# VaibhavKamat/Performance-Comparison-of-TensorFlow-PyTorch-and-their-Distributed-Counterparts

Hardware: AMD Instinct MI355X
Metric: resnet50_train_images_per_sec (higher is better)
Workload: dtype bf16; 1 GPU; model=resnet50, global_batch=256, per_gpu_batch=256, image_size=224, num_classes=1000, parallelism=dp1, impl=hip, optimizer=sgd_momentum, hipgraph=False, ddp_force=False, grad_allreduce_dtype=fp32, lr_warmup_steps=5

## Files before the change

performance-comparison-of-tensorflow-pytorch-and-their-distributed-counterparts_amd/csrc/bnr_stream.h:

```cpp
#pragma once
#include "igemm.h"

namespace pcmp {

inline Knob kn_bnr_stream("bnr_stream", 1);
inline Knob kn_bnr_stream_wgs("bnr_stream_wgs", 256);

template <int BN, int GK, bool FOLD, bool DUAL>
__global__ void __launch_bounds__(256, 2) bnr_stream_kernel(const IgemmParams p, int groups) {
  constexpr int BM = 32, NTHR = 256;
  constexpr int KB = GK / 64;
  constexpr int A_IMG = BM * GK * 2;
  constexpr int STAGE = A_IMG * (FOLD ? 2 : 1);
  constexpr int W_BYTES = BN * GK * 2;
  constexpr int CS = BN + 8;
  constexpr int C_BYTES = BM * CS * 4;
  constexpr int CPR = BN / 8;
  constexpr int NCH = BM * BN / 8 / NTHR;
  constexpr int RPP = NTHR / CPR;
  constexpr int NS = DUAL ? 3 : 2;
  constexpr int NWT = BN / 32;
  constexpr int NAI = A_IMG / 1024 / 4;
  constexpr int NWI = W_BYTES / 1024 / 4;
  constexpr int NEL = NCH * (DUAL ? 4 : 3);
// ... 212 lines not shown
        u &= mfx ? kz : kbits;
        const float g0 = __uint_as_float(u << 16), g1 = __uint_as_float(u & 0xffff0000u);
        sm[0][2 * q] += g0;
        sm[0][2 * q + 1] += g1;
        sm[1][2 * q] += g0 * fmaf(xa, ka[2 * q], kb[2 * q]);
        sm[1][2 * q + 1] += g1 * fmaf(xb, ka[2 * q + 1], kb[2 * q + 1]);
        if constexpr (DUAL) {
          const unsigned x2w = q == 0 ? eX2[S][k].x : q == 1 ? eX2[S][k].y : q == 2 ? eX2[S][k].z : eX2[S][k].w;
          sm[2][2 * q] += g0 * fmaf(__uint_as_float(x2w << 16), ka2[2 * q], kb2[2 * q]);
          sm[2][2 * q + 1] += g1 * fmaf(__uint_as_float(x2w & 0xffff0000u), ka2[2 * q + 1], kb2[2 * q + 1]);
        }
        ov[q] = u;
      }
      const size_t o = (size_t)(pt * BM + row) * p.gn + n0 + c8 * 8;
      *reinterpret_cast<uint4*>(out + o) = uint4{ov[0], ov[1], ov[2], ov[3]};
    }
  };
  int j = 0;
  for (; j + 1 < nmine; j += 2) {
    tile(std::integral_constant<int, 0>{}, j);
    tile(std::integral_constant<int, 1>{}, j + 1);
  }
  if (j < nmine) tile(std::integral_constant<int, 0>{}, j);

  __syncthreads();
  float* red = reinterpret_cast<float*>(sS);
#pragma unroll
  for (int q = 0; q < NS; ++q) {
    *reinterpret_cast<f32x4*>(red + (r0 * NS + q) * BN + c8 * 8) = f32x4{sm[q][0], sm[q][1], sm[q][2], sm[q][3]};
    *reinterpret_cast<f32x4*>(red + (r0 * NS + q) * BN + c8 * 8 + 4) = f32x4{sm[q][4], sm[q][5], sm[q][6], sm[q][7]};
  }
  __syncthreads();
  for (int i = tid; i < NS * BN; i += NTHR) {
    const int q = i / BN, c = i - q * BN;
    float t = 0.f;
    for (int r = 0; r < RPP; ++r) t += red[(r * NS + q) * BN + c];
    float* st = p.stats + (size_t)grp * 2 * p.gn;
    if (q == 0) {
      st[n0 + c] = t;
      if constexpr (DUAL) p.stats2[(size_t)grp * 2 * p.gn + n0 + c] = t;
    } else if (q == 1) {
      st[p.gn + n0 + c] = t;
    } else {
      p.stats2[(size_t)grp * 2 * p.gn + p.gn + n0 + c] = t;
    }
  }
}

static bool use_bnr_stream(const IgemmParams& p) {
  if (!kn_bnr_stream.get() || !p.bn_x || p.R != 1 || p.S != 1 || p.stride != 1 || p.pad != 0) return false;
  if (!(p.gk == 64 || p.gk == 128 || p.gk == 256) || p.gn % 64 || p.gm % 32) return false;
  if (!p.bn_mbits && !(p.bn_msc && !p.bn_mask)) return false;
  if (p.relu) return false;
  if ((p.fold_x ? 2 : 1) * p.gk >= p.gn) return false;
  return (int64_t)p.gm * p.gn * 2 < (1ll << 31) && (int64_t)p.gm * p.gk * 2 < (1ll << 31);
}

static int bnr_stream_bn(const IgemmParams& p) { return p.gn == 64 ? 64 : 128; }

static int bnr_stream_groups(const IgemmParams& p) {
  const int ntn = p.gn / bnr_stream_bn(p);
  const int npt = p.gm / 32;
  return std::max(1, std::min(npt, std::max(1, kn_bnr_stream_wgs.get() / ntn)));
}

template <int BN, int GK, bool FOLD, bool DUAL>
static void launch_bnr_stream_cfg(IgemmParams& p, hipStream_t st) {
  constexpr int BM = 32;
  const int ntn = p.gn / BN;
  const int groups = bnr_stream_groups(p);
  TORCH_CHECK(p.stats && p.stats_cap >= groups && (!DUAL || p.stats2), "bnr_stream: partial-stats buffers");
  constexpr size_t stage = (size_t)BM * GK * 2 * (FOLD ? 2 : 1);
  constexpr size_t red = (size_t)(256 / (BN / 8)) * (DUAL ? 3 : 2) * BN * 4;
  constexpr size_t body = 2 * stage + (size_t)BM * (BN + 8) * 4 + (FOLD ? 3 * GK * 4 : 0);
  constexpr size_t smem = (size_t)BN * GK * 2 + std::max(body, red);
  static_assert(smem <= 160 * 1024, "bnr_stream: LDS");
  launch_lds<bnr_stream_kernel<BN, GK, FOLD, DUAL>>(dim3(groups * ntn), dim3(256), smem, st, p, groups);
}

static void launch_bnr_stream(IgemmParams& p, hipStream_t st) {
  const bool fold = p.fold_x != nullptr, dual = p.bn_x2 != nullptr;
  const int BN = bnr_stream_bn(p);
#define PCMP_BNRS(B, G)                                                                      \
  do {                                                                                      \
    if (fold) {                                                                             \
      if (dual) launch_bnr_stream_cfg<B, G, true, true>(p, st);                             \
      else launch_bnr_stream_cfg<B, G, true, false>(p, st);                                 \
    } else {                                                                                \
      if (dual) launch_bnr_stream_cfg<B, G, false, true>(p, st);                            \
      else launch_bnr_stream_cfg<B, G, false, false>(p, st);                                \
    }                                                                                       \
  } while (0)
  if (BN == 64) {
    if (p.gk == 64) PCMP_BNRS(64, 64); else if (p.gk == 128) PCMP_BNRS(64, 128); else PCMP_BNRS(64, 256);
  } else {
    if (p.gk == 64) PCMP_BNRS(128, 64); else if (p.gk == 128) PCMP_BNRS(128, 128); else PCMP_BNRS(128, 256);
  }
#undef PCMP_BNRS
}

}

namespace pcmp {

inline Knob kn_fwd_stream("fwd_stream", 1);
inline Knob kn_fwd_stream_wgs("fwd_stream_wgs", 512);

// ... 214 lines not shown
```

performance-comparison-of-tensorflow-pytorch-and-their-distributed-counterparts_amd/csrc/igemm.h:

```cpp
#pragma once
#include "igemm_plan.h"

namespace pcmp {

static unsigned tensor_bytes(const at::Tensor& t) {
  const int64_t b = t.numel() * t.element_size();
  TORCH_CHECK(b < (1ll << 31), "igemm: operand larger than 2 GiB (buffer-resource range)");
  return (unsigned)b;
}

static void fill_geometry(IgemmParams& p, int N, int H, int W, int C, int K, int R, int S,
                          int stride, int pad) {
  p.N = N; p.H = H; p.W = W; p.C = C; p.K = K; p.R = R; p.S = S;
  p.stride = stride; p.pad = pad;
  p.P = (H + 2 * pad - R) / stride + 1;
  p.Q = (W + 2 * pad - S) / stride + 1;
  p.fd_PQ = make_fastdiv(p.P * p.Q);
  p.fd_Q = make_fastdiv(p.Q);
  p.fd_HW = make_fastdiv(H * W);
  p.fd_W = make_fastdiv(W);
  p.dH = H; p.dW = W; p.offy = pad; p.offx = pad; p.sub = 0; p.oph = 0; p.opw = 0;
  p.bias = nullptr; p.resid = nullptr; p.aux = nullptr; p.stats = nullptr; p.stats2 = nullptr;
  p.bn_mask = nullptr; p.bn_x = nullptr; p.bn_mean = nullptr; p.bn_istd = nullptr;
  p.bn_x2 = nullptr; p.bn_mean2 = nullptr; p.bn_istd2 = nullptr; p.bn_msc = nullptr; p.bn_msh = nullptr;
  p.bn_mbits = nullptr;
  p.stats_cap = 0;
  p.relu = 0; p.alpha = 1.f; p.accumulate = 0; p.nsplit = 1;
  p.fold_x = nullptr; p.fold_coef = nullptr; p.fold_lds = 0;
  p.act_sc = nullptr; p.act_sh = nullptr;
  p.resid_sub = 0; p.rs_H2 = 0; p.rs_W2 = 0;
}

std::vector<at::Tensor> conv_fwd(const at::Tensor& x, const at::Tensor& w, int64_t stride, int64_t pad,
                                 const c10::optional<at::Tensor>& bias,
                                 const c10::optional<at::Tensor>& resid, bool relu, bool want_stats,
                                 const c10::optional<at::Tensor>& in_scale, const c10::optional<at::Tensor>& in_shift);
std::vector<std::string> plan_candidates(const at::Tensor& x, const at::Tensor& w, int64_t stride, int64_t pad,
                                         const c10::optional<at::Tensor>& bias, const c10::optional<at::Tensor>& resid,
                                         bool relu);
std::vector<at::Tensor> linear_gelu_fwd(const at::Tensor& x, const at::Tensor& w, const c10::optional<at::Tensor>& bias);
at::Tensor conv_dgrad(const at::Tensor& dy, const at::Tensor& w, int64_t H, int64_t W, int64_t stride, int64_t pad,
                      const c10::optional<at::Tensor>& resid, const c10::optional<at::Tensor>& wt);
at::Tensor linear_dgrad_gelu(const at::Tensor& dy, const at::Tensor& w, const at::Tensor& u,
                             const c10::optional<at::Tensor>& wt);
std::vector<at::Tensor> conv_dgrad_bnr(const at::Tensor& dy, const at::Tensor& w, int64_t H, int64_t W,
                                       int64_t stride, int64_t pad, const c10::optional<at::Tensor>& resid,
                                       const c10::optional<at::Tensor>& ymask, const at::Tensor& x,
                                       const at::Tensor& mean, const at::Tensor& invstd,
                                       const c10::optional<at::Tensor>& x2, const c10::optional<at::Tensor>& mean2,
                                       const c10::optional<at::Tensor>& invstd2, const c10::optional<at::Tensor>& mscale,
                                       const c10::optional<at::Tensor>& mshift, const c10::optional<at::Tensor>& wt,
                                       const c10::optional<at::Tensor>& ymask_bits,
                                       const c10::optional<at::Tensor>& fold_x,
                                       const c10::optional<at::Tensor>& fold_coef, bool resid_sub);
void conv_wgrad(const at::Tensor& dy, const at::Tensor& x, at::Tensor out, int64_t R, int64_t S,
                int64_t stride, int64_t pad, bool accumulate, const c10::optional<at::Tensor>& fold_x,
                const c10::optional<at::Tensor>& fold_coef, const c10::optional<at::Tensor>& in_scale,
                const c10::optional<at::Tensor>& in_shift);
std::vector<at::Tensor> conv1x1_bwd_fused(const at::Tensor& g, const c10::optional<at::Tensor>& fold_x,
                                          const c10::optional<at::Tensor>& fold_coef, const at::Tensor& wt,
                                          const at::Tensor& z, const at::Tensor& scale, const at::Tensor& shift,
                                          const at::Tensor& mean, const at::Tensor& invstd, at::Tensor dw,
                                          bool accumulate);

}
```

performance-comparison-of-tensorflow-pytorch-and-their-distributed-counterparts_amd/csrc/igemm_dgrad.hip:

```cpp
#include "igemm.h"
#include "bnr_stream.h"
#include "bwd_fused.h"

namespace pcmp {

static at::Tensor transpose_taps(const at::Tensor& w, int r0, int s0, int rstep, int subR, int subS,
                                 hipStream_t st) {
  const int K = w.size(0), R = w.size(1), S = w.size(2), C = w.size(3);
  auto wt = at::empty({C, subR, subS, K}, w.options());
  dim3 grid(ceil_div(C, 64), ceil_div(K, 64), subR * subS);
  hipLaunchKernelGGL(wt_transpose_kernel, grid, dim3(256), 0, st, ptr<unsigned short>(w), ptr<unsigned short>(wt), K,
                     R, S, C, r0, s0, rstep, subS, subR * subS);
  PCMP_LAUNCH_CHECK();
  return wt;
}

struct BnrArgs {
  const __bf16* fold_x = nullptr;
  const float* fold_coef = nullptr;
  const uint8_t* mbits = nullptr;
  const __bf16* mask = nullptr;
  const __bf16* x = nullptr;
  const float* mean = nullptr;
  const float* istd = nullptr;
// ... 59 lines not shown
    for (int oph = 0; oph < 2; ++oph)
      for (int opw = 0; opw < 2; ++opw) {
        const int r0 = (oph + pad) & 1, s0 = (opw + pad) & 1;
        const int subR = r0 < R ? (R - r0 + 1) / 2 : 0, subS = s0 < S ? (S - s0 + 1) / 2 : 0;
        const int dH = (H - oph + 1) / 2, dW = (W - opw + 1) / 2;
        if (dH <= 0 || dW <= 0) continue;
        if (subR == 0 || subS == 0) {
          TORCH_CHECK(!bn, "conv_dgrad_bnr: stride-2 filter leaves pixel classes uncovered");
          uncovered = true;
          continue;
        }
        cls.push_back({oph, opw, r0, s0, subR, subS, dH, dW});
      }
    const bool accum = has_res || uncovered;
    at::Tensor dx = has_res ? *resid : (uncovered ? at::zeros({N, H, W, C}, dy.options())
                                                  : at::empty({N, H, W, C}, dy.options()));
    auto class_params = [&](const Cls& c, const at::Tensor& wt) {
      IgemmParams q = p;
      q.R = c.subR; q.S = c.subS;
      q.sub = 1; q.oph = c.oph; q.opw = c.opw;
      q.dH = c.dH; q.dW = c.dW;
      q.fd_HW = make_fastdiv(c.dH * c.dW);
      q.fd_W = make_fastdiv(c.dW);
      q.offy = (c.oph + pad - c.r0) / 2;
      q.offx = (c.opw + pad - c.s0) / 2;
      q.gm = N * c.dH * c.dW; q.gn = C; q.gk = c.subR * c.subS * K;
      q.a = ptr<__bf16>(dy); q.out = dx.data_ptr();
      q.a_bytes = tensor_bytes(dy);
      if (wt.defined()) { q.b = ptr<__bf16>(wt); q.b_bytes = tensor_bytes(wt); }
      q.resid = accum ? ptr<__bf16>(dx) : nullptr;
      q.ksplit = q.gk;
      set_bn(q);
      return q;
    };
    at::Tensor part, part2;
    if (bn) {
      int T = 0;
      for (auto& c : cls) {
        const IgemmParams q = class_params(c, at::Tensor());
        T += ceil_div(q.gm, igemm_bm(MODE_DGRAD, q));
      }
      part = at::empty({T, 2, C}, fopts);
      if (two) part2 = at::empty({T, 2, C}, fopts);
    }
    int64_t cls_off[2][2] = {{0, 0}, {0, 0}}, cls_total = 0;
    for (int oph = 0; oph < 2; ++oph)
      for (int opw = 0; opw < 2; ++opw) {
        const int r0 = (oph + pad) & 1, s0 = (opw + pad) & 1;
        const int subR = r0 < R ? (R - r0 + 1) / 2 : 0, subS = s0 < S ? (S - s0 + 1) / 2 : 0;
        cls_off[oph][opw] = cls_total;
        cls_total += (int64_t)C * subR * subS * K;
      }
    TORCH_CHECK(!wt_cls.defined() || cls_total == wt_cls.numel(), "conv_dgrad: class-blocked weight size");
    int toff = 0;
    for (auto& c : cls) {
      const bool whole = c.subR == R && c.subS == S && wt_full.defined();
      at::Tensor wt = wt_cls.defined()
                          ? wt_cls.narrow(0, cls_off[c.oph][c.opw], (int64_t)C * c.subR * c.subS * K)
                                .view({C, c.subR, c.subS, K})
                          : (whole ? wt_full : transpose_taps(w, c.r0, c.s0, 2, c.subR, c.subS, st));
      IgemmParams q = class_params(c, wt);
      if (bn) {
        q.stats = ptr<float>(part) + (size_t)toff * 2 * C;
        if (two) q.stats2 = ptr<float>(part2) + (size_t)toff * 2 * C;
        q.stats_cap = (int)part.size(0) - toff;
        toff += ceil_div(q.gm, igemm_bm(MODE_DGRAD, q));
      }
      dispatch<MODE_DGRAD>(q, st);
    }
    if (!bn) return {dx};
    if (two) return {dx, part, part2};
    return {dx, part};
  }
  at::Tensor wt = wt_full.defined() ? wt_full : transpose_taps(w, 0, 0, 1, R, S, st);
  auto dx = at::empty({N, H, W, C}, dy.options());
  p.gm = N * H * W; p.gn = C; p.gk = R * S * K;
  p.a = ptr<__bf16>(dy); p.b = ptr<__bf16>(wt); p.out = dx.data_ptr();
  p.a_bytes = tensor_bytes(dy); p.b_bytes = tensor_bytes(wt);
  if (has_res) p.resid = ptr<__bf16>(*resid);
  if (dgelu_u) {
    TORCH_CHECK(!has_res && !bn && stride == 1 && R == 1 && S == 1, "linear_dgrad_gelu: plain 1x1 GEMM only");
    PCMP_CHECK_BF16(*dgelu_u); PCMP_CHECK_CONTIG(*dgelu_u);
    TORCH_CHECK(dgelu_u->numel() == (int64_t)N * H * W * C, "linear_dgrad_gelu: u shape");
    p.resid = ptr<__bf16>(*dgelu_u);
    p.relu = 3;
  }
  p.ksplit = p.gk;
  if (!bn && plain_gemm_eligible<MODE_DGRAD>(p)) {
    const GemmPlan pl = plan_gemm<MODE_DGRAD>(p, ptr<__bf16>(dx), fopts, st);
    run_plan<MODE_DGRAD>(p, pl, ptr<__bf16>(dx), fopts, st);
    return {dx};
  }
  at::Tensor part, part2;
  if (bn) {
    set_bn(p);
    if (use_bnr_stream(p)) {
      const int T = bnr_stream_groups(p);
      part = at::empty({T, 2, C}, fopts);
      p.stats_cap = T;
      p.stats = ptr<float>(part);
      if (two) { part2 = at::empty({T, 2, C}, fopts); p.stats2 = ptr<float>(part2); }
      launch_bnr_stream(p, st);
      if (two) return {dx, part, part2};
      return {dx, part};
    }
    const int T = ceil_div(p.gm, igemm_bm(MODE_DGRAD, p));
    part = at::empty({T, 2, C}, fopts);
    p.stats_cap = T;
    p.stats = ptr<float>(part);
    if (two) { part2 = at::empty({T, 2, C}, fopts); p.stats2 = ptr<float>(part2); }
  }
  dispatch<MODE_DGRAD>(p, st);
  if (!bn) return {dx};
  if (two) return {dx, part, part2};
  return {dx, part};
}

at::Tensor conv_dgrad(const at::Tensor& dy, const at::Tensor& w, int64_t H, int64_t W, int64_t stride,
                      int64_t pad, const c10::optional<at::Tensor>& resid, const c10::optional<at::Tensor>& wt) {
  if (dy.scalar_type() == at::kFloat) return f32::conv_dgrad(dy, w, H, W, stride, pad, resid);
  return dgrad_impl(dy, w, H, W, stride, pad, resid, nullptr, wt)[0];
}
// ... 111 lines not shown
```

performance-comparison-of-tensorflow-pytorch-and-their-distributed-counterparts_amd/csrc/igemm_kernels.h:

```cpp
#pragma once
#include "common.h"
#include "f32.h"

#include <algorithm>
#include <string>
#include <vector>

namespace pcmp {

struct FastDiv {
  uint32_t d, m, s;
};
static FastDiv make_fastdiv(uint32_t d) {
  FastDiv f;
  f.d = d;
  uint32_t s = 0;
  while ((1ull << s) < d) ++s;
  f.s = s;
  f.m = (uint32_t)(((1ull << 32) * ((1ull << s) - d)) / d + 1);
  return f;
}
__device__ __forceinline__ uint32_t fdiv(uint32_t n, const FastDiv& f) {
  return (__umulhi(n, f.m) + n) >> f.s;
}

enum IgemmMode { MODE_FWD = 0, MODE_DGRAD = 1, MODE_WGRAD = 2 };

struct IgemmParams {
  const __bf16* a;
  const __bf16* b;
  void* out;
  const float* bias;
  const __bf16* resid;
  __bf16* aux;
  float* stats;
  int gm, gn, gk;
  int N, H, W, C, K, R, S, P, Q, stride, pad;
  FastDiv fd_PQ, fd_Q, fd_HW, fd_W;
  int dH, dW, offy, offx, sub, oph, opw;
  int relu;
  unsigned a_bytes, b_bytes;
  int ksplit;
  int nsplit;
  int tiles_m, tiles_n;
  float alpha;
  int accumulate;
  const __bf16* bn_mask;
  const __bf16* bn_x;
  const float* bn_mean;
  const float* bn_istd;
  const __bf16* bn_x2;
  const float* bn_mean2;
  const float* bn_istd2;
  float* stats2;
  const float* bn_msc;
  const float* bn_msh;
  const uint8_t* bn_mbits;
  int stats_cap;
  const __bf16* fold_x;
  const float* fold_coef;
  int fold_lds;
  const float* act_sc;
  const float* act_sh;
  int resid_sub, rs_H2, rs_W2;
};

__device__ __forceinline__ uint4 fold_act(uint4 z, const float* a, const float* b, bool ok) {
  const u16x8 zv = __builtin_bit_cast(u16x8, z);
  u16x8 o;
#pragma unroll
  for (int e = 0; e < 8; ++e) o[e] = ok ? f2bf(fmaxf(bf2f(zv[e]) * a[e] + b[e], 0.f)) : (unsigned short)0;
  return __builtin_bit_cast(uint4, o);
}

__device__ __forceinline__ uint4 fold_dz(uint4 g, uint4 x, const float* k1, const float* k2, const float* k3,
                                         bool ok) {
  const u16x8 gv = __builtin_bit_cast(u16x8, g), xv = __builtin_bit_cast(u16x8, x);
  u16x8 o;
#pragma unroll
  for (int e = 0; e < 8; ++e) o[e] = ok ? f2bf(k1[e] * bf2f(gv[e]) + k2[e] * bf2f(xv[e]) + k3[e]) : (unsigned short)0;
  return __builtin_bit_cast(uint4, o);
}

constexpr int BK = 64;
constexpr int NT = 256;

inline Knob kn_wgrad_m32("wgrad_m32", 1);
inline Knob kn_epi_depth("epi_depth", 4);
inline Knob kn_epi_depth_bnr2("epi_depth_bnr2", 2);

__device__ __forceinline__ int xcd_remap(int bid, int nwg) {
  if (nwg <= 8) return bid;
  const int xcd = bid & 7, q = nwg >> 3, r = nwg & 7;
  const int base = (xcd < r) ? xcd * (q + 1) : r * (q + 1) + (xcd - r) * q;
  return base + (bid >> 3);
}

__device__ __forceinline__ int rr_off(int row, int chunk) {
  return row * (BK * 2) + ((chunk ^ (row & 7)) << 4);
}

template <int COLS, bool M32 = false>
__device__ __forceinline__ int tr_off(int row, int col) {
  constexpr int RB = COLS * 2;
  int x;
  if constexpr (M32) {
    if constexpr (RB >= 256) x = 4 * (row & 3);
    else if constexpr (RB == 128) x = 4 * ((row >> 1) & 1);
    else x = 0;
  } else {
    int f;
    if constexpr (RB >= 256) {
      f = (row & 3) | (((row >> 3) & 1) << 2);
    } else if constexpr (RB == 128) {
      f = ((row >> 1) & 1) | (((row >> 3) & 1) << 1);
    } else {
      f = 0;
// ... 774 lines not shown
      if (kt + 1 < nk) store_stage(cur ^ 1);
      __syncthreads();
    }
  }

  const int fr = lane & 15, fq = lane >> 4;
  if constexpr (M32) {
    float* out = reinterpret_cast<float*>(p.out) + (size_t)split * p.gm * p.gn;
#pragma unroll
    for (int i = 0; i < TM32; ++i)
#pragma unroll
      for (int j = 0; j < TN32; ++j) {
        const int col = n0 + wc * WTN + j * 32 + (lane & 31);
#pragma unroll
        for (int r = 0; r < 16; ++r) {
          const int row = m0 + wr * WTM + i * 32 + 8 * (r >> 2) + 4 * (lane >> 5) + (r & 3);
          if (row < p.gm && col < p.gn) {
            float v = acc32[i][j][r] * p.alpha;
            float* dst = out + (size_t)row * p.gn + col;
            if (p.accumulate) v += *dst;
            *dst = v;
          }
        }
      }
    return;
  } else if constexpr (MODE == MODE_WGRAD) {
    float* out = reinterpret_cast<float*>(p.out) + (size_t)split * p.gm * p.gn;
#pragma unroll
    for (int i = 0; i < TM; ++i)
#pragma unroll
      for (int j = 0; j < TN; ++j) {
        const int col = n0 + wc * WTN + j * 16 + fr;
#pragma unroll
        for (int e = 0; e < 4; ++e) {
          const int row = m0 + wr * WTM + i * 16 + fq * 4 + e;
          if (row < p.gm && col < p.gn) {
            float v = acc[i][j][e] * p.alpha;
            float* dst = out + (size_t)row * p.gn + col;
            if (p.accumulate) v += *dst;
            *dst = v;
          }
        }
      }
    return;
  } else {
    igemm_epilogue_fd<MODE, BM, BN, WM, WN, EPI, NTHR, EPD>(p, acc, smem, tid, m0, n0, tile_m, split);
  }
}

constexpr int NT8 = 512;
constexpr int BM8 = 256;


template <int MODE, int BM, int BN, int WM, int WN, int NTHR, int MINB, int EPI, int EPD = 2>
__global__ void __launch_bounds__(NTHR, MINB) igemm_dma_kernel(const IgemmParams p) {
  constexpr int NW = NTHR / 64;
  constexpr int WTM = BM / WM, WTN = BN / WN;
  constexpr int TM = WTM / 16, TN = WTN / 16;
  constexpr int TMH = TM / 2, TNH = TN / 2;
  constexpr int A_BYTES = BM * BK * 2, B_BYTES = BN * BK * 2;
  constexpr int STAGE = A_BYTES + B_BYTES;
  constexpr int NA = BM / 16 / NW;
  constexpr int NB = BN / 16 / NW;
  constexpr int AH = WTM / 2, BH = WTN / 2;
  static_assert(MODE != MODE_WGRAD, "FWD/DGRAD only");
  static_assert(WM * WN == NW, "one wave tile per wave");
  static_assert(NA >= 1 && NB >= 1 && NA * NW * 16 == BM && NB * NW * 16 == BN, "loader slots");
  static_assert(AH % 8 == 0 && BH % 8 == 0 && TM % 2 == 0 && TN % 2 == 0, "quadrants");
  static_assert(WTN % 32 == 0, "PAIR channel permutation works on 32-row groups");

  extern __shared__ __attribute__((aligned(16))) char smem[];
  const int tid = threadIdx.x, lane = tid & 63, wid = tid >> 6;
  const int wr = wid / WN, wc = wid % WN;

  const int lin = xcd_remap(blockIdx.x, gridDim.x);
  const int tiles_mn = p.tiles_m * p.tiles_n;
  const int split = lin / tiles_mn;
  const int tl = lin - split * tiles_mn;
  const int tile_n = tl % p.tiles_n;
  const int tile_m = tl / p.tiles_n;
  const int m0 = tile_m * BM, n0 = tile_n * BN;
  const int kbeg = split * p.ksplit;
  const int nk = (min(p.gk, kbeg + p.ksplit) - kbeg) / BK;

  f32x4 acc[TN][TM];
#pragma unroll
  for (int j = 0; j < TN; ++j)
#pragma unroll
    for (int i = 0; i < TM; ++i) acc[j][i] = f32x4{0.f, 0.f, 0.f, 0.f};

  const __amdgpu_buffer_rsrc_t rsA = make_rsrc(p.a, p.a_bytes);
  const __amdgpu_buffer_rsrc_t rsB = make_rsrc(p.b, p.b_bytes);

  const int gch = (lane & 7) ^ (lane >> 3);
  int a_off[2][NA], a_y[2][NA], a_x[2][NA], a_lds[2][NA];
  int b_off[2][NB], b_lds[2][NB];
#pragma unroll
  for (int mh = 0; mh < 2; ++mh)
#pragma unroll
    for (int i = 0; i < NA; ++i) {
      const int h0 = wid * (8 * NA) + i * 8;
      const int row0 = (h0 / AH) * WTM + mh * AH + h0 % AH;
      a_lds[mh][i] = row0 * (BK * 2);
      const int m = m0 + row0 + (lane >> 3);
      const bool v = m < p.gm;
      const int mm = v ? m : 0;
      if constexpr (MODE == MODE_FWD) {
        const int n = fdiv(mm, p.fd_PQ);
        const int rem = mm - n * p.P * p.Q;
        const int pp = fdiv(rem, p.fd_Q);
        const int qq = rem - pp * p.Q;
        const int yv = pp * p.stride - p.pad;
        a_y[mh][i] = v ? yv : -(1 << 28);
        a_x[mh][i] = qq * p.stride - p.pad;
        a_off[mh][i] = ((n * p.H + yv) * p.W + a_x[mh][i]) * p.C + gch * 8;
      } else {
        const int n = fdiv(mm, p.fd_HW);
        const int rem = mm - n * p.dH * p.dW;
        const int hh = fdiv(rem, p.fd_W);
        const int ww = rem - hh * p.dW;
        const int yv = hh + p.offy;
        a_y[mh][i] = v ? yv : -(1 << 28);
        a_x[mh][i] = ww + p.offx;
        a_off[mh][i] = ((n * p.P + yv) * p.Q + a_x[mh][i]) * p.K + gch * 8;
      }
    }
#pragma unroll
  for (int nh = 0; nh < 2; ++nh)
// ... 68 lines not shown
    for (int kk = 0; kk < 2; ++kk)
#pragma unroll
      for (int j = 0; j < TNH; ++j)
#pragma unroll
        for (int i = 0; i < TMH; ++i)
          acc[nh * TNH + j][mh * TMH + i] =
              __builtin_amdgcn_mfma_f32_16x16x32_bf16(fb[nh][j][kk], fa[i][kk], acc[nh * TNH + j][mh * TMH + i], 0, 0, 0);
  };

  struct KS { int k0, kc, ks, kr; };
  auto adv = [&](KS st) {
    st.k0 += BK; st.kc += BK;
    if (st.kc >= CIN) { st.kc = 0; if (++st.ks == p.S) { st.ks = 0; ++st.kr; } }
    return st;
  };
  auto set_state = [&](const KS& st) { k0 = st.k0; kc = st.kc; ks = st.ks; kr = st.kr; };
  const KS s0{k0, kc, ks, kr};
  KS s1 = adv(s0), s2 = adv(s1);
  issue_a(0, 0); issue_b(0, 0); issue_b(1, 0); issue_a(1, 0);
  if (nk > 1) {
    set_state(s1);
    issue_a(0, 1); issue_b(1, 1); issue_a(1, 1);
    wait_vm<2 * NA + NB>();
  } else {
    wait_vm<0>();
  }
  lds_barrier();
  for (int t = 0; t < nk; ++t) {
    const int buf = t & 1, nb = buf ^ 1;
    const bool has1 = t + 1 < nk, has2 = t + 2 < nk;
    read_a(0, buf); read_b(0, buf);
    if (has1) { set_state(s1); issue_b(0, nb); }
    mma(0, 0);
    lds_sync();
    read_b(1, buf);
    if (has2) { set_state(s2); issue_a(0, buf); }
    mma(0, 1);
    lds_sync();
    read_a(1, buf);
    if (has2) issue_b(1, buf);
    mma(1, 1);
    lds_sync();
    read_b(0, buf);
    if (has2) issue_a(1, buf);
    mma(1, 0);
    if (has2) wait_vm<2 * NA + NB>(); else wait_vm<0>();
    lds_sync();
    s1 = s2;
    s2 = adv(s2);
  }
  igemm_epilogue_fd<MODE, BM, BN, WM, WN, EPI, NTHR, EPD>(p, acc, smem, tid, m0, n0, tile_m, split);
}

template <int N>
__device__ __forceinline__ void wait_vm_b() {
  static_assert(N >= 0 && N < 64, "vmcnt");
  __builtin_amdgcn_s_waitcnt((N & 15) | ((N >> 4) << 14) | (7 << 4) | (15 << 8));
}
__device__ __forceinline__ void lds_sync_b() {
  __builtin_amdgcn_s_waitcnt(15 | (3 << 14) | (7 << 4));
  __builtin_amdgcn_s_barrier();
}
__device__ __forceinline__ int chan_perm32(int rho) {
  return (rho & ~31) | (((rho >> 2) & 1) << 4) | (((rho >> 3) & 3) << 2) | (rho & 3);
}

__device__ __forceinline__ float row16_transpose_sum(const float (&v)[16], int lane) {
  const bool b3 = lane & 8, b2 = lane & 4, b1 = lane & 2, b0 = lane & 1;
  float w[8], x[4], y[2];
#pragma unroll
  for (int k = 0; k < 8; ++k) w[k] = (b3 ? v[k + 8] : v[k]) + dpp_mov<0x140>(b3 ? v[k] : v[k + 8]);
#pragma unroll
  for (int k = 0; k < 4; ++k) x[k] = (b2 ? w[k + 4] : w[k]) + dpp_mov<0x141>(b2 ? w[k] : w[k + 4]);
#pragma unroll
  for (int k = 0; k < 2; ++k) y[k] = (b1 ? x[k + 2] : x[k]) + dpp_mov<0x4E>(b1 ? x[k] : x[k + 2]);
  return (b0 ? y[1] : y[0]) + dpp_mov<0xB1>(b0 ? y[0] : y[1]);
}

template <int MODE, int BM, int BN, int WM, int WN, int EPI, int EPD>
__device__ __forceinline__ void igemm_epilogue32(const IgemmParams& p, f32x16 (&acc)[BN / WN / 32][BM / WM / 32],
                                                 const float* ctab, float* red, int tid, int m0, int n0, int tile_m) {
  constexpr int WTM = BM / WM, WTN = BN / WN;
  constexpr int TM = WTM / 32, TN = WTN / 32;
  constexpr int NTH = 256;
  constexpr int NI = TN * TM * 2;
  constexpr int IPJ = TM * 2;
  constexpr bool stats = EPI == EPI_STATS;
  constexpr bool bnr = MODE == MODE_DGRAD && (EPI == EPI_BNR || EPI == EPI_BNR2);
  constexpr bool bnr2 = MODE == MODE_DGRAD && EPI == EPI_BNR2;
  constexpr int NS = bnr2 ? 3 : 2;
  static_assert(EPI != EPI_GELU, "igemm_epilogue32: conv epilogues only");
  const int lane = tid & 63, wid = tid >> 6;
  const int wr = wid / WN, wc = wid % WN;
  const int h = lane >> 5, pr = lane & 31;
  __bf16* out = reinterpret_cast<__bf16*>(p.out);
  const bool has_res = p.resid != nullptr;
  const bool has_mb = bnr && p.bn_mbits != nullptr;
  const bool has_mk = bnr && !has_mb && p.bn_mask != nullptr;
  const bool mfx = bnr && !has_mb && !has_mk && p.bn_msc != nullptr;
  const bool has_bias = MODE == MODE_FWD && p.bias != nullptr;
  size_t orows[TM];
  int rrows[MODE == MODE_DGRAD ? TM : 1];
#pragma unroll
  for (int i = 0; i < TM; ++i) {
    const int m = m0 + wr * WTM + i * 32 + pr;
    size_t orow = m < p.gm ? m : 0;
// ... 1077 lines not shown
```

performance-comparison-of-tensorflow-pytorch-and-their-distributed-counterparts_amd/csrc/igemm_launch.h:

```cpp
#pragma once
#include "igemm_kernels.h"

namespace pcmp {

template <int MODE>
static int epi_of(const IgemmParams& p) {
  if (MODE == MODE_FWD && p.stats) return EPI_STATS;
  if (MODE == MODE_DGRAD && p.bn_x) return p.bn_x2 ? EPI_BNR2 : EPI_BNR;
  return MODE != MODE_WGRAD && p.relu >= 2 ? EPI_GELU : EPI_PLAIN;
}

template <int MODE, int BN, int WM, int WN, int NW = 4>
static size_t epi_scratch_bytes(const IgemmParams& p) {
  if (!((MODE == MODE_FWD && p.stats) || (MODE == MODE_DGRAD && p.bn_x))) return 0;
  const int NS = MODE == MODE_DGRAD && p.bn_x2 ? 3 : 2;
  return (size_t)(NW * 16 * (NS * (BN / WN) + 4) + WM * NS * BN) * sizeof(float);
}

template <int MODE, int BM, int BN, int WM, int WN, int FOLD, int E, int D = 2>
static void launch_igemm(bool unif, int grid, size_t smem, hipStream_t st, const IgemmParams& p) {
  if constexpr (FOLD != 0) {
    launch_lds<igemm_kernel<MODE, BM, BN, WM, WN, true, E, D, NT, FOLD>>(dim3(grid), dim3(NT), smem, st, p);
  } else {
    if (unif) launch_lds<igemm_kernel<MODE, BM, BN, WM, WN, true, E, D>>(dim3(grid), dim3(NT), smem, st, p);
// ... 302 lines not shown
      if (p.fold_x) {
        if (p.gn <= 64) launch_cfg<MODE, 128, 64, 2, 2, 3>(p, st); else launch_cfg<MODE, 128, 128, 2, 2, 3>(p, st);
      } else {
        if (p.gn <= 64) launch_cfg<MODE, 128, 64, 2, 2, 2>(p, st); else launch_cfg<MODE, 128, 128, 2, 2, 2>(p, st);
      }
      return;
    }
    if (wgrad_wide(p) == 1) launch_cfg<MODE, 64, 256, 1, 4, 1>(p, st);
    else if (p.gm <= 64) {
      if (p.gn <= 64) launch_cfg<MODE, 64, 64, 2, 2, 1>(p, st); else launch_cfg<MODE, 64, 128, 2, 2, 1>(p, st);
    } else {
      if (p.gn <= 64) launch_cfg<MODE, 128, 64, 2, 2, 1>(p, st); else launch_cfg<MODE, 128, 128, 2, 2, 1>(p, st);
    }
  }
}

template <int MODE>
static void dispatch(IgemmParams& p, hipStream_t st) {
  if (p.fold_x || p.act_sc) { launch_fold<MODE>(p, st); return; }
  if constexpr (MODE != MODE_WGRAD) {
    if (use_halo(MODE, p)) { launch_halo<MODE>(p, st); return; }
    if (use_igemm8(MODE, p) == 256) { launch_dma<MODE, 256, 256, 2, 4, NT8, 1>(p, st); return; }
  }
  if constexpr (MODE == MODE_WGRAD) {
    const int w = wgrad_wide(p);
    if (w == 1) { launch_cfg<MODE, 64, 256, 1, 4>(p, st); return; }
    if (w == 2) { launch_cfg<MODE, 256, 64, 4, 1>(p, st); return; }
  }
  if constexpr (MODE != MODE_WGRAD) {
    if (use_bm64_smallgrid(MODE, p)) { launch_cfg<MODE, 64, 128, 2, 2>(p, st); return; }
    switch (use_dma4(MODE, p)) {
      case 1:
        if (use_dma32(MODE, p)) launch_dma32<MODE, 128, 128, 2, 2>(p, st); else launch_dma<MODE, 128, 128, 2, 2, NT, 2>(p, st);
        return;
      case 2:
        if (use_dma32(MODE, p)) launch_dma32<MODE, 128, 64, 2, 2>(p, st); else launch_dma<MODE, 128, 64, 2, 2, NT, 2>(p, st);
        return;
      case 3: launch_dma<MODE, 256, 64, 4, 1, NT, 2>(p, st); return;
      default: break;
    }
  }
  if (p.gm <= 32) {
    if (p.gn <= 64) launch_cfg<MODE, 32, 64, 1, 4>(p, st);
    else launch_cfg<MODE, 32, 128, 1, 4>(p, st);
  } else if (p.gm <= 64) {
    if (p.gn <= 64) launch_cfg<MODE, 64, 64, 2, 2>(p, st);
    else launch_cfg<MODE, 64, 128, 2, 2>(p, st);
  } else {
    if (p.gn <= 64) launch_cfg<MODE, 128, 64, 2, 2>(p, st);
    else launch_cfg<MODE, 128, 128, 2, 2>(p, st);
  }
}

template <int BM, int BN, int WM, int WN, int MINB>
static void launch_gemm32(IgemmParams& p, hipStream_t st) {
  TORCH_CHECK(p.R == 1 && p.S == 1 && p.stride == 1 && p.pad == 0 && p.gk % BK == 0 && p.ksplit % BK == 0 &&
                  !p.stats && !p.bn_x && !p.fold_x && !p.act_sc && p.gn % 4 == 0,
              "gemm32: plain 1x1 GEMMs only");
  p.tiles_m = ceil_div(p.gm, BM);
  p.tiles_n = ceil_div(p.gn, BN);
  const int grid = p.tiles_m * p.tiles_n * p.nsplit;
  constexpr size_t smem = (size_t)2 * (BM + BN) * BK * 2;
  static_assert(smem <= 160 * 1024, "gemm32: LDS budget");
  launch_lds<gemm32_kernel<BM, BN, WM, WN, MINB>>(dim3(grid), dim3(WM * WN * 64), smem, st, p);
}

template <class T>
static void launch_splitk_reduce2(const T* ws, T* out, int n4, int nsplit, bool accumulate, hipStream_t st) {
  const int SL = nsplit <= 8 ? 1 : (nsplit <= 32 ? 4 : 16);
  const dim3 grid(ceil_div(n4, 256 / SL)), block(256);
  if (SL == 1) hipLaunchKernelGGL(splitk_reduce2_kernel<1>, grid, block, 0, st, ws, out, n4, nsplit, (int)accumulate);
  else if (SL == 4) hipLaunchKernelGGL(splitk_reduce2_kernel<4>, grid, block, 0, st, ws, out, n4, nsplit, (int)accumulate);
  else hipLaunchKernelGGL(splitk_reduce2_kernel<16>, grid, block, 0, st, ws, out, n4, nsplit, (int)accumulate);
  PCMP_LAUNCH_CHECK();
}

}
```

Baseline: 13970 images/s.

## Merge strided dgrad sub-pixel class GEMMs into one multi-class DMA launch

For strided convolution dgrad, the sub-pixel tap classes were each dispatched as a separate GEMM kernel. This groups classes sharing the same DMA tile config and output geometry into a single launch with a per-class parameter table, so blocks pick their class from blockIdx. The goal is fewer launches and a fuller grid, since each class alone is a small GEMM. It also loosens the bnr_stream eligibility check for the fold path (2*gk == gn now allowed), which adds another case to that kernel and enlarges IgemmParams with the class table.

```diff
diff --git a/performance-comparison-of-tensorflow-pytorch-and-their-distributed-counterparts_amd/csrc/bnr_stream.h b/performance-comparison-of-tensorflow-pytorch-and-their-distributed-counterparts_amd/csrc/bnr_stream.h
--- a/performance-comparison-of-tensorflow-pytorch-and-their-distributed-counterparts_amd/csrc/bnr_stream.h
+++ b/performance-comparison-of-tensorflow-pytorch-and-their-distributed-counterparts_amd/csrc/bnr_stream.h
@@ -288,7 +288,7 @@
   if (!(p.gk == 64 || p.gk == 128 || p.gk == 256) || p.gn % 64 || p.gm % 32) return false;
   if (!p.bn_mbits && !(p.bn_msc && !p.bn_mask)) return false;
   if (p.relu) return false;
-  if ((p.fold_x ? 2 : 1) * p.gk >= p.gn) return false;
+  if (p.fold_x ? 2 * p.gk > p.gn : p.gk >= p.gn) return false;
   return (int64_t)p.gm * p.gn * 2 < (1ll << 31) && (int64_t)p.gm * p.gk * 2 < (1ll << 31);
 }
 
diff --git a/performance-comparison-of-tensorflow-pytorch-and-their-distributed-counterparts_amd/csrc/igemm.h b/performance-comparison-of-tensorflow-pytorch-and-their-distributed-counterparts_amd/csrc/igemm.h
--- a/performance-comparison-of-tensorflow-pytorch-and-their-distributed-counterparts_amd/csrc/igemm.h
+++ b/performance-comparison-of-tensorflow-pytorch-and-their-distributed-counterparts_amd/csrc/igemm.h
@@ -29,6 +29,7 @@
   p.fold_x = nullptr; p.fold_coef = nullptr; p.fold_lds = 0;
   p.act_sc = nullptr; p.act_sh = nullptr;
   p.resid_sub = 0; p.rs_H2 = 0; p.rs_W2 = 0;
+  p.ncls = 0;
 }
 
 std::vector<at::Tensor> conv_fwd(const at::Tensor& x, const at::Tensor& w, int64_t stride, int64_t pad,
diff --git a/performance-comparison-of-tensorflow-pytorch-and-their-distributed-counterparts_amd/csrc/igemm_dgrad.hip b/performance-comparison-of-tensorflow-pytorch-and-their-distributed-counterparts_amd/csrc/igemm_dgrad.hip
--- a/performance-comparison-of-tensorflow-pytorch-and-their-distributed-counterparts_amd/csrc/igemm_dgrad.hip
+++ b/performance-comparison-of-tensorflow-pytorch-and-their-distributed-counterparts_amd/csrc/igemm_dgrad.hip
@@ -135,6 +135,8 @@
         cls_total += (int64_t)C * subR * subS * K;
       }
     TORCH_CHECK(!wt_cls.defined() || cls_total == wt_cls.numel(), "conv_dgrad: class-blocked weight size");
+    struct Run { IgemmParams q; at::Tensor wt; int tile, row0; bool merged; };
+    std::vector<Run> runs;
     int toff = 0;
     for (auto& c : cls) {
       const bool whole = c.subR == R && c.subS == S && wt_full.defined();
@@ -143,14 +145,41 @@
                                 .view({C, c.subR, c.subS, K})
                           : (whole ? wt_full : transpose_taps(w, c.r0, c.s0, 2, c.subR, c.subS, st));
       IgemmParams q = class_params(c, wt);
+      const int row0 = toff;
       if (bn) {
         q.stats = ptr<float>(part) + (size_t)toff * 2 * C;
         if (two) q.stats2 = ptr<float>(part2) + (size_t)toff * 2 * C;
         q.stats_cap = (int)part.size(0) - toff;
         toff += ceil_div(q.gm, igemm_bm(MODE_DGRAD, q));
       }
-      dispatch<MODE_DGRAD>(q, st);
-    }
+      runs.push_back({q, wt, kn_dgrad_s2_merge.get() ? dgrad_dma_tile(q) : 0, row0, false});
+    }
+    for (size_t i = 0; i < runs.size(); ++i) {
+      if (runs[i].merged || !runs[i].tile) continue;
+      std::vector<Run*> grp;
+      for (size_t j = i; j < runs.size(); ++j)
+        if (!runs[j].merged && runs[j].tile == runs[i].tile && runs[j].q.dH == runs[i].q.dH && runs[j].q.dW == runs[i].q.dW)
+          grp.push_back(&runs[j]);
+      if (grp.size() < 2) continue;
+      std::stable_sort(grp.begin(), grp.end(), [](const Run* a, const Run* b) { return a->q.gk > b->q.gk; });
+      IgemmParams m = grp[0]->q;
+      m.ncls = (int)grp.size();
+      if (bn) {
+        m.stats = ptr<float>(part);
+        if (two) m.stats2 = ptr<float>(part2);
+        m.stats_cap = (int)part.size(0);
+      }
+      for (int k = 0; k < m.ncls; ++k) {
+        const IgemmParams& q = grp[k]->q;
+        m.cls[k] = DgradCls{q.b, q.b_bytes, q.R, q.S, q.offy, q.offx, q.oph, q.opw, q.gk, 0, grp[k]->row0};
+        grp[k]->merged = true;
+      }
+      if (runs[i].tile == 8) launch_dma_cls<256, 256, 2, 4, NT8, 1>(m, st);
+      else if (runs[i].tile == 1) launch_dma_cls<128, 128, 2, 2, NT, 2>(m, st);
+      else launch_dma_cls<128, 64, 2, 2, NT, 2>(m, st);
+    }
+    for (auto& r : runs)
+      if (!r.merged) dispatch<MODE_DGRAD>(r.q, st);
     if (!bn) return {dx};
     if (two) return {dx, part, part2};
     return {dx, part};
diff --git a/performance-comparison-of-tensorflow-pytorch-and-their-distributed-counterparts_amd/csrc/igemm_kernels.h b/performance-comparison-of-tensorflow-pytorch-and-their-distributed-counterparts_amd/csrc/igemm_kernels.h
--- a/performance-comparison-of-tensorflow-pytorch-and-their-distributed-counterparts_amd/csrc/igemm_kernels.h
+++ b/performance-comparison-of-tensorflow-pytorch-and-their-distributed-counterparts_amd/csrc/igemm_kernels.h
@@ -25,6 +25,14 @@
 }
 
 enum IgemmMode { MODE_FWD = 0, MODE_DGRAD = 1, MODE_WGRAD = 2 };
+
+struct DgradCls {
+  const __bf16* b;
+  unsigned b_bytes;
+  int R, S, offy, offx, oph, opw, gk;
+  int tile0;
+  int row0;
+};
 
 struct IgemmParams {
   const __bf16* a;
@@ -63,6 +71,8 @@
   const float* act_sc;
   const float* act_sh;
   int resid_sub, rs_H2, rs_W2;
+  int ncls;
+  DgradCls cls[4];
 };
 
 __device__ __forceinline__ uint4 fold_act(uint4 z, const float* a, const float* b, bool ok) {
@@ -943,8 +953,8 @@
 constexpr int BM8 = 256;
 
 
-template <int MODE, int BM, int BN, int WM, int WN, int NTHR, int MINB, int EPI, int EPD = 2>
-__global__ void __launch_bounds__(NTHR, MINB) igemm_dma_kernel(const IgemmParams p) {
+template <int MODE, int BM, int BN, int WM, int WN, int NTHR, int EPI, int EPD>
+__device__ __forceinline__ void igemm_dma_tile(const IgemmParams& p, const int lin) {
   constexpr int NW = NTHR / 64;
   constexpr int WTM = BM / WM, WTN = BN / WN;
   constexpr int TM = WTM / 16, TN = WTN / 16;
@@ -964,7 +974,6 @@
   const int tid = threadIdx.x, lane = tid & 63, wid = tid >> 6;
   const int wr = wid / WN, wc = wid % WN;
 
-  const int lin = xcd_remap(blockIdx.x, gridDim.x);
   const int tiles_mn = p.tiles_m * p.tiles_n;
   const int split = lin / tiles_mn;
   const int tl = lin - split * tiles_mn;
@@ -1139,6 +1148,39 @@
   igemm_epilogue_fd<MODE, BM, BN, WM, WN, EPI, NTHR, EPD>(p, acc, smem, tid, m0, n0, tile_m, split);
 }
 
+template <int MODE, int BM, int BN, int WM, int WN, int NTHR, int MINB, int EPI, int EPD = 2>
+__global__ void __launch_bounds__(NTHR, MINB) igemm_dma_kernel(const IgemmParams p) {
+  igemm_dma_tile<MODE, BM, BN, WM, WN, NTHR, EPI, EPD>(p, xcd_remap(blockIdx.x, gridDim.x));
+}
+
+template <int BM, int BN, int WM, int WN, int NTHR, int MINB, int EPI, int EPD = 2>
+__global__ void __launch_bounds__(NTHR, MINB) igemm_dma_cls_kernel(const IgemmParams pin) {
+  const int bid = blockIdx.x;
+  DgradCls k = pin.cls[0];
+  int ntile = pin.ncls > 1 ? pin.cls[1].tile0 : (int)gridDim.x;
+#pragma unroll
+  for (int i = 1; i < 4; ++i)
+    if (i < pin.ncls && bid >= pin.cls[i].tile0) {
+      k = pin.cls[i];
+      ntile = (i + 1 < pin.ncls ? pin.cls[i + 1 < 4 ? i + 1 : 3].tile0 : (int)gridDim.x) - k.tile0;
+    }
+  IgemmParams p = pin;
+  p.R = __builtin_amdgcn_readfirstlane(k.R);
+  p.S = __builtin_amdgcn_readfirstlane(k.S);
+  p.offy = __builtin_amdgcn_readfirstlane(k.offy);
+  p.offx = __builtin_amdgcn_readfirstlane(k.offx);
+  p.oph = __builtin_amdgcn_readfirstlane(k.oph);
+  p.opw = __builtin_amdgcn_readfirstlane(k.opw);
+  p.gk = p.ksplit = __builtin_amdgcn_readfirstlane(k.gk);
+  p.b = k.b;
+  p.b_bytes = (unsigned)__builtin_amdgcn_readfirstlane((int)k.b_bytes);
+  const int row0 = __builtin_amdgcn_readfirstlane(k.row0);
+  if (p.stats) p.stats += (size_t)row0 * 2 * p.gn;
+  if (EPI == EPI_BNR2) p.stats2 += (size_t)row0 * 2 * p.gn;
+  const int tile0 = __builtin_amdgcn_readfirstlane(k.tile0);
+  igemm_dma_tile<MODE_DGRAD, BM, BN, WM, WN, NTHR, EPI, EPD>(p, xcd_remap(bid - tile0, ntile));
+}
+
 template <int N>
 __device__ __forceinline__ void wait_vm_b() {
   static_assert(N >= 0 && N < 64, "vmcnt");
diff --git a/performance-comparison-of-tensorflow-pytorch-and-their-distributed-counterparts_amd/csrc/igemm_launch.h b/performance-comparison-of-tensorflow-pytorch-and-their-distributed-counterparts_amd/csrc/igemm_launch.h
--- a/performance-comparison-of-tensorflow-pytorch-and-their-distributed-counterparts_amd/csrc/igemm_launch.h
+++ b/performance-comparison-of-tensorflow-pytorch-and-their-distributed-counterparts_amd/csrc/igemm_launch.h
@@ -378,6 +378,48 @@
   }
 }
 
+inline Knob kn_dgrad_s2_merge("dgrad_s2_merge", 1);
+
+static int dgrad_dma_tile(const IgemmParams& p) {
+  if (p.fold_x || p.act_sc || p.relu >= 2 || use_halo(MODE_DGRAD, p)) return 0;
+  if (use_igemm8(MODE_DGRAD, p) == 256) return 8;
+  if (use_bm64_smallgrid(MODE_DGRAD, p)) return 0;
+  const int v = use_dma4(MODE_DGRAD, p);
+  return (v == 1 || v == 2) && !use_dma32(MODE_DGRAD, p) ? v : 0;
+}
+
+template <int BM, int BN, int WM, int WN, int NTHR, int MINB, int E>
+static void launch_dma_cls_epi(int grid, size_t smem, hipStream_t st, const IgemmParams& p) {
+  constexpr bool can_deep = (E == EPI_BNR || E == EPI_BNR2) && NTHR == 256;
+  if (can_deep && (E == EPI_BNR2 ? kn_epi_depth_bnr2 : kn_epi_depth).get() >= 4)
+    launch_lds<igemm_dma_cls_kernel<BM, BN, WM, WN, NTHR, MINB, E, 4>>(dim3(grid), dim3(NTHR), smem, st, p);
+  else
+    launch_lds<igemm_dma_cls_kernel<BM, BN, WM, WN, NTHR, MINB, E, 2>>(dim3(grid), dim3(NTHR), smem, st, p);
+}
+
+template <int BM, int BN, int WM, int WN, int NTHR, int MINB>
+static void launch_dma_cls(IgemmParams& p, hipStream_t st) {
+  p.tiles_m = ceil_div(p.gm, BM);
+  p.tiles_n = ceil_div(p.gn, BN);
+  TORCH_CHECK(p.ncls >= 2 && p.ncls <= 4 && p.sub && p.nsplit == 1 && p.K % BK == 0, "igemm_dma_cls: class table");
+  for (int i = 0; i < p.ncls; ++i) {
+    TORCH_CHECK(p.cls[i].gk % BK == 0 && p.cls[i].gk >= BK, "igemm_dma_cls: needs the block-uniform tap walk");
+    TORCH_CHECK(!p.stats || p.cls[i].row0 + p.tiles_m <= p.stats_cap, "igemm_dma_cls: partial-stats buffer too small");
+    p.cls[i].tile0 = i * p.tiles_m * p.tiles_n;
+  }
+  const int grid = p.ncls * p.tiles_m * p.tiles_n;
+  const size_t smem = std::max((size_t)2 * (BM + BN) * BK * 2, epi_scratch_bytes<MODE_DGRAD, BN, WM, WN, NTHR / 64>(p));
+  const int epi = epi_of<MODE_DGRAD>(p);
+  if (epi == EPI_BNR) launch_dma_cls_epi<BM, BN, WM, WN, NTHR, MINB, EPI_BNR>(grid, smem, st, p);
+  else if (epi == EPI_BNR2) {
+    if constexpr (NTHR == 256) launch_dma_cls_epi<BM, BN, WM, WN, NTHR, MINB, EPI_BNR2>(grid, smem, st, p);
+    else TORCH_CHECK(false, "igemm8: dual BN-reduce epilogue not instantiated");
+  } else {
+    TORCH_CHECK(epi == EPI_PLAIN, "igemm_dma_cls: conv epilogues only");
+    launch_dma_cls_epi<BM, BN, WM, WN, NTHR, MINB, EPI_PLAIN>(grid, smem, st, p);
+  }
+}
+
 template <int BM, int BN, int WM, int WN, int MINB>
 static void launch_gemm32(IgemmParams& p, hipStream_t st) {
   TORCH_CHECK(p.R == 1 && p.S == 1 && p.stride == 1 && p.pad == 0 && p.gk % BK == 0 && p.ksplit % BK == 0 &&
```

After: 14090 images/s, median of 6. Within noise of the previous version (+0.9%).
